# cliangyu/video-diffusion

Measured on AMD Instinct MI355X. Metric: denoise-steps/sec, higher is better.
Workload: dtype f32

## Files before the change

### video-diffusion_amd/csrc/attn_temporal.hip

```cpp
#include "vd_common.h"
#include <cstdlib>
#include <string>

namespace vd {

__device__ __forceinline__ float dot4(f32x4 a, f32x4 b) { return a.x * b.x + a.y * b.y + a.z * b.z + a.w * b.w; }

template <int PB, int TMAX, bool RPE>
__global__ __launch_bounds__(256) void attn_temporal_kernel(AttnTemporalArgs a) {
    extern __shared__ __attribute__((aligned(16))) float smem[];
    const int T = a.T, C = a.C, HW = a.HW, C3 = 3 * a.C;
    const int F = C / a.heads, F4 = F >> 2, FP = F + 4, TS = T + 1;
    float* qs = smem;
    float* ks = qs + PB * T * FP;
    float* sc = ks + PB * T * FP;
    const int b = blockIdx.z, h = blockIdx.y, p0 = blockIdx.x * PB;
    const int np = min(PB, HW - p0);
    const int tid = threadIdx.x;
    const float* qkv_b = a.qkv + (size_t)b * T * HW * C3 + h * F;

    for (int idx = tid; idx < PB * T * F4; idx += 256) {
        const int f4 = idx % F4, r = idx / F4;
        const int t = r % T, p = r / T;
        const float* src = qkv_b + ((size_t)t * HW + p0 + min(p, np - 1)) * C3 + f4 * 4;
        f32x4 q = *reinterpret_cast<const f32x4*>(src) * a.scale;
        f32x4 k = *reinterpret_cast<const f32x4*>(src + C);
        if (p >= np) { q = f32x4{0.f, 0.f, 0.f, 0.f}; k = q; }
        *reinterpret_cast<f32x4*>(qs + (p * T + t) * FP + f4 * 4) = q;
        *reinterpret_cast<f32x4*>(ks + (p * T + t) * FP + f4 * 4) = k;
    }
    __syncthreads();

    for (int pr = tid; pr < T * T; pr += 256) {
        const int t = pr / T, s = pr - t * T;
        float acc[PB];
#pragma unroll
        for (int p = 0; p < PB; ++p) acc[p] = 0.f;
        const float* rk = RPE ? a.Rk + (((size_t)b * T + t) * T + s) * C + h * F : nullptr;
        const float* rq = RPE ? a.Rq + (((size_t)b * T + s) * T + t) * C + h * F : nullptr;
        const float* qrow = qs + t * FP;
        const float* krow = ks + s * FP;
#pragma unroll 3
        for (int f0 = 0; f0 < F; f0 += 8) {
            f32x4 rk0, rk1, rq0, rq1;
            if constexpr (RPE) {
                rk0 = *reinterpret_cast<const f32x4*>(rk + f0); rk1 = *reinterpret_cast<const f32x4*>(rk + f0 + 4);
                rq0 = *reinterpret_cast<const f32x4*>(rq + f0) * a.scale; rq1 = *reinterpret_cast<const f32x4*>(rq + f0 + 4) * a.scale;
            }
#pragma unroll
            for (int p = 0; p < PB; ++p) {
                const f32x4 q0 = *reinterpret_cast<const f32x4*>(qrow + p * T * FP + f0);
                const f32x4 q1 = *reinterpret_cast<const f32x4*>(qrow + p * T * FP + f0 + 4);
                const f32x4 k0 = *reinterpret_cast<const f32x4*>(krow + p * T * FP + f0);
                const f32x4 k1 = *reinterpret_cast<const f32x4*>(krow + p * T * FP + f0 + 4);
                if constexpr (RPE)
                    acc[p] += dot4(q0, k0 + rk0) + dot4(q1, k1 + rk1) + dot4(k0, rq0) + dot4(k1, rq1);
                else
                    acc[p] += dot4(q0, k0) + dot4(q1, k1);
            }
        }
        bool masked = false;
        if (a.mask) {
            const float mt = a.mask[b * T + t], ms = a.mask[b * T + s];
            float allowed = mt * ms;
            if (a.allow_pad) allowed += (1.f - mt) * (1.f - ms);
            else if (t == s) allowed = 1.f;
            masked = allowed == 0.f;
        }
#pragma unroll
        for (int p = 0; p < PB; ++p) sc[(p * T + t) * TS + s] = masked ? -INFINITY : acc[p];
    }
    __syncthreads();

    for (int row = tid; row < np * T; row += 256) {
        float* r = sc + row * TS;
        float mx = -INFINITY;
        for (int s = 0; s < T; ++s) mx = fmaxf(mx, r[s]);
        float sum = 0.f;
        for (int s = 0; s < T; ++s) { const float e = __expf(r[s] - mx); r[s] = e; sum += e; }
        const float inv = 1.0f / sum;
        for (int s = 0; s < T; ++s) r[s] *= inv;
    }
    __syncthreads();

    for (int item = tid; item < T * F4; item += 256) {
        const int t = item / F4, f4 = item - t * F4;
        f32x4 rv[TMAX];
#pragma unroll
        for (int s = 0; s < TMAX; ++s) {
            rv[s] = f32x4{0.f, 0.f, 0.f, 0.f};
            if constexpr (RPE)
                rv[s] = *reinterpret_cast<const f32x4*>(a.Rv + (((size_t)b * T + t) * T + min(s, T - 1)) * C + h * F + f4 * 4);
        }
        for (int p = 0; p < np; ++p) {
            const float* ar = sc + (p * T + t) * TS;
            const float* vbase = qkv_b + 2 * C + (size_t)(p0 + p) * C3 + f4 * 4;
            f32x4 o = {0.f, 0.f, 0.f, 0.f};
#pragma unroll
            for (int s = 0; s < TMAX; ++s) {
                const f32x4 v = *reinterpret_cast<const f32x4*>(vbase + (size_t)min(s, T - 1) * HW * C3);
                const float w = s < T ? ar[min(s, T - 1)] : 0.f;
                o += (v + rv[s]) * w;
            }
            *reinterpret_cast<f32x4*>(a.out + (((size_t)b * T + t) * HW + p0 + p) * C + h * F + f4 * 4) = o;
        }
    }
}

#ifdef VD_ATT_TIMING
__device__ unsigned long long g_att_stamp[16];
#define ATT_STAMP(i)                                                                                   \
    do {                                                                                               \
        if (threadIdx.x == 0 && blockIdx.x == 3 && blockIdx.y == 1 && blockIdx.z == 2) {               \
            __builtin_amdgcn_sched_barrier(0);                                                         \
            g_att_stamp[i] = __builtin_amdgcn_s_memrealtime();                                         \
            __builtin_amdgcn_sched_barrier(0);                                                         \
        }                                                                                              \
    } while (0)
extern "C" int vd_debug_att_stamps(unsigned long long* host_out) {
    return (int)hipMemcpyFromSymbol(host_out, HIP_SYMBOL(g_att_stamp), sizeof(g_att_stamp));
}
#else
#define ATT_STAMP(i)
#endif

__device__ __forceinline__ f32x4 mfma4(float x, float y, f32x4 c) { return __builtin_amdgcn_mfma_f32_16x16x4f32(x, y, c, 0, 0, 0); }

__device__ __forceinline__ void rows_regs_transpose(float& x0, float& x1, float& x2, float& x3) {
    auto u = [](float f) { return __builtin_bit_cast(unsigned, f); };
    auto f = [](unsigned v) { return __builtin_bit_cast(float, v); };
    auto p01 = __builtin_amdgcn_permlane16_swap(u(x0), u(x1), false, false);
    auto p23 = __builtin_amdgcn_permlane16_swap(u(x2), u(x3), false, false);
    auto q02 = __builtin_amdgcn_permlane32_swap(p01[0], p23[0], false, false);
    auto q13 = __builtin_amdgcn_permlane32_swap(p01[1], p23[1], false, false);
    x0 = f(q02[0]); x2 = f(q02[1]); x1 = f(q13[0]); x3 = f(q13[1]);
}

template <int NT, int JM, bool RPE, bool EXACT>
__global__ __launch_bounds__(512, 2) void attn_temporal_mfma_kernel(AttnTemporalArgs a) {
    constexpr int TP = 16 * NT, RS = TP + 1, PS = TP * RS + (NT == 1 ? 1 : 17);
    extern __shared__ __attribute__((aligned(16))) float smem[];
    float* w = smem;
    const int T = EXACT ? 16 * NT : a.T, C = a.C, HW = a.HW, C3 = 3 * a.C;
    const int F = C / a.heads, NJ = EXACT ? JM : F >> 4;
    const int b = blockIdx.z, h = blockIdx.y, p0 = blockIdx.x * 16;
    const int tid = threadIdx.x, wv = tid >> 6, l = tid & 63, i16 = l & 15, g = l >> 4;
    const float* qb = a.qkv + ((size_t)b * T * HW + p0) * C3 + h * F;
    auto row = [&](int t, int px) { return qb + ((size_t)t * HW + px) * C3; };
    auto ld4 = [](const float* p) { return *reinterpret_cast<const f32x4*>(p); };
    const int tcl[2] = {min(i16, T - 1), min(16 + i16, T - 1)};
    const f32x4 zero4 = {0.f, 0.f, 0.f, 0.f};

    ATT_STAMP(0);
    constexpr int JG = NT == 1 ? 2 : 1, NG = JM / JG, NU = 2 * NT;
    constexpr bool AHEAD = NT == 1;
    struct Ops { f32x4 qa1[2][NT][JG], kb1[2][NT][JG], xa2[NU][JG], rb2[NU][NT][JG], xa3[NU][JG], rb3[NU][NT][JG]; };
    f32x4 acc1[2][NT][NT], acc2[NU][NT], acc3[NU][NT];
#pragma unroll
    for (int u = 0; u < 2; ++u)
#pragma unroll
        for (int m = 0; m < NT; ++m)
#pragma unroll
            for (int n = 0; n < NT; ++n) acc1[u][m][n] = zero4;
#pragma unroll
    for (int u = 0; u < NU; ++u)
#pragma unroll
        for (int n = 0; n < NT; ++n) { acc2[u][n] = zero4; acc3[u][n] = zero4; }
    const float* q1[2][NT];
#pragma unroll
    for (int u = 0; u < 2; ++u)
#pragma unroll
        for (int m = 0; m < NT; ++m) q1[u][m] = row(tcl[m], 2 * wv + u) + 4 * g;
    const float* rkq[NT];
#pragma unroll
    for (int n = 0; n < NT; ++n) rkq[n] = (size_t)b * T * T * C + (size_t)tcl[n] * C + h * F + 4 * g + (const float*)nullptr;
    auto request = [&](Ops& o, int grp, bool own, bool rel) {
#pragma unroll
        for (int jj = 0; jj < JG; ++jj) {
            const int j = grp * JG + jj;
            if (EXACT || j < NJ) {
                if (own) {
#pragma unroll
                    for (int u = 0; u < 2; ++u)
#pragma unroll
                        for (int m = 0; m < NT; ++m) { o.qa1[u][m][jj] = ld4(q1[u][m] + 16 * j); o.kb1[u][m][jj] = ld4(q1[u][m] + C + 16 * j); }
                }
                if constexpr (RPE) {
#pragma unroll
                    for (int u = 0; u < (rel ? NU : 0); ++u) {
                        const int t = wv + 8 * u;
                        if (EXACT || t < T) {
                            const float* xr = row(t, i16) + 4 * g + 16 * j;
                            o.xa2[u][jj] = ld4(xr);
                            o.xa3[u][jj] = ld4(xr + C);
#pragma unroll
                            for (int n = 0; n < NT; ++n) {
                                const size_t ro = (size_t)(rkq[n] - (const float*)nullptr) + (size_t)t * T * C + 16 * j;
                                o.rb2[u][n][jj] = ld4(a.Rk + ro);
                                o.rb3[u][n][jj] = ld4(a.Rq + ro);
                            }
                        }
                    }
                }
            }
        }
    };
    auto products = [&](const Ops& o, int grp, bool own, bool rel) {
#pragma unroll
        for (int jj = 0; jj < JG; ++jj) {
            if (EXACT || grp * JG + jj < NJ) {
#pragma unroll
                for (int e = 0; e < 4; ++e) {
#pragma unroll
                    for (int u = 0; u < (own ? 2 : 0); ++u)
#pragma unroll
                        for (int m = 0; m < NT; ++m)
#pragma unroll
                            for (int n = 0; n < NT; ++n) acc1[u][m][n] = mfma4(o.qa1[u][m][jj][e] * a.scale, o.kb1[u][n][jj][e], acc1[u][m][n]);
                    if constexpr (RPE) {
#pragma unroll
                        for (int u = 0; u < (rel ? NU : 0); ++u)
                            if (EXACT || wv + 8 * u < T) {
#pragma unroll
                                for (int n = 0; n < NT; ++n) {
                                    acc2[u][n] = mfma4(o.xa2[u][jj][e] * a.scale, o.rb2[u][n][jj][e], acc2[u][n]);
                                    acc3[u][n] = mfma4(o.xa3[u][jj][e], o.rb3[u][n][jj][e] * a.scale, acc3[u][n]);
                                }
                            }
                    }
                }
            }
        }
    };
    if constexpr (AHEAD) {
        Ops o[2];
        request(o[0], 0, true, true);
#pragma unroll
        for (int grp = 0; grp < NG; ++grp) {
            if (grp + 1 < NG) request(o[(grp + 1) & 1], grp + 1, true, true);
            __builtin_amdgcn_sched_barrier(0);
            products(o[grp & 1], grp, true, true);
            __builtin_amdgcn_sched_barrier(0);
        }
    } else {
#pragma unroll 1
        for (int grp = 0; grp < NG; ++grp) {
            Ops o;
            request(o, grp, true, false);
            products(o, grp, true, false);
            if constexpr (RPE) {
                request(o, grp, false, true);
                products(o, grp, false, true);
            }
        }
    }
    ATT_STAMP(1);
#pragma unroll
    for (int u = 0; u < 2; ++u)
#pragma unroll
        for (int m = 0; m < NT; ++m)
#pragma unroll
            for (int n = 0; n < NT; ++n)
#pragma unroll
                for (int r = 0; r < 4; ++r) w[(2 * wv + u) * PS + (16 * m + 4 * g + r) * RS + 16 * n + i16] = acc1[u][m][n][r];
    __syncthreads();
    if constexpr (RPE) {
#pragma unroll
        for (int u = 0; u < NU; ++u) {
            const int t = wv + 8 * u;
            if (t < T) {
#pragma unroll
                for (int n = 0; n < NT; ++n)
#pragma unroll
                    for (int r = 0; r < 4; ++r) w[(4 * g + r) * PS + t * RS + 16 * n + i16] += acc2[u][n][r];
            }
        }
        __syncthreads();
#pragma unroll
        for (int u = 0; u < NU; ++u) {
            const int sk = wv + 8 * u;
            if (sk < T) {
#pragma unroll
                for (int n = 0; n < NT; ++n)
#pragma unroll
                    for (int r = 0; r < 4; ++r) w[(4 * g + r) * PS + (16 * n + i16) * RS + sk] += acc3[u][n][r];
            }
        }
        __syncthreads();
    }

    ATT_STAMP(2);
    for (int rix = tid; rix < 16 * TP; rix += 512) {
        const int px = rix / TP, t = rix - px * TP;
        float* r = w + px * PS + t * RS;
        if (t >= T) {
            for (int s = 0; s < TP; ++s) r[s] = 0.f;
            continue;
        }
        float mx = -INFINITY;
        const float mt = a.mask ? a.mask[b * T + t] : 1.f;
        for (int s = 0; s < T; ++s) {
            float v = r[s];
            if (a.mask) {
                const float ms = a.mask[b * T + s];
                float allowed = mt * ms;
                if (a.allow_pad) allowed += (1.f - mt) * (1.f - ms);
                else if (t == s) allowed = 1.f;
                if (allowed == 0.f) v = -INFINITY;
            }
            r[s] = v;
            mx = fmaxf(mx, v);
        }
        float sum = 0.f;
        for (int s = 0; s < T; ++s) { const float e = __expf(r[s] - mx); r[s] = e; sum += e; }
        const float inv = 1.0f / sum;
        for (int s = 0; s < T; ++s) r[s] *= inv;
        for (int s = T; s < TP; ++s) r[s] = 0.f;
    }
    __syncthreads();

    ATT_STAMP(3);
    const int KS = (T + 3) >> 2;
    if (EXACT ? wv < JM : wv < NJ) {
        const int f0 = 16 * wv + i16;
        const float* vb = qb + 2 * C + f0;
        const float* rvb = RPE ? a.Rv + ((size_t)b * T) * T * C + h * F + f0 : nullptr;
#pragma unroll 1
        for (int m = 0; m < NT; ++m) {
            if (16 * m >= T) break;
            float rr[NT == 1 ? 4 : 1][16];
            f32x4 acc[16];
#pragma unroll
            for (int px = 0; px < 16; ++px) acc[px] = zero4;
#pragma unroll 1
            for (int kc = 0; kc < NT; ++kc) {
                if (16 * kc >= T) break;
                float vr[4][16];
#pragma unroll
                for (int k4 = 0; k4 < 4; ++k4)
                    if (EXACT || 4 * kc + k4 < KS) {
                        const float* vs = vb + (size_t)min(16 * kc + 4 * k4 + g, T - 1) * HW * C3;
#pragma unroll
                        for (int px = 0; px < 16; ++px) vr[k4][px] = vs[(size_t)px * C3];
                    }
                if constexpr (RPE && NT == 1) {
#pragma unroll
                    for (int k4 = 0; k4 < 4; ++k4)
                        if (EXACT || k4 < KS) {
                            const float* rv = rvb + (size_t)min(4 * k4 + g, T - 1) * C;
#pragma unroll
                            for (int tl = 0; tl < 16; ++tl) rr[k4][tl] = rv[(size_t)min(tl, T - 1) * T * C];
                        }
                }
                __builtin_amdgcn_sched_barrier(0);
#pragma unroll
                for (int k4 = 0; k4 < 4; ++k4)
                    if (EXACT || 4 * kc + k4 < KS) {
                        const float* ar = w + (16 * m + i16) * RS + 16 * kc + 4 * k4 + g;
#pragma unroll
                        for (int px = 0; px < 16; ++px) acc[px] = mfma4(ar[px * PS], vr[k4][px], acc[px]);
                    }
            }
            ATT_STAMP(4);
            f32x4 res[16];
#pragma unroll
            for (int bq = 0; bq < 4; ++bq)
#pragma unroll
                for (int d = 0; d < 4; ++d) {
                    float x0 = acc[bq][d], x1 = acc[4 + bq][d], x2 = acc[8 + bq][d], x3 = acc[12 + bq][d];
                    rows_regs_transpose(x0, x1, x2, x3);
                    res[d][bq] = x0; res[4 + d][bq] = x1; res[8 + d][bq] = x2; res[12 + d][bq] = x3;
                }
            if constexpr (RPE) {
                if constexpr (NT == 1) {
#pragma unroll
                    for (int k4 = 0; k4 < 4; ++k4)
                        if (EXACT || k4 < KS) {
                            const float* ar = w + i16 * PS + 4 * k4 + g;
#pragma unroll
                            for (int tl = 0; tl < 16; ++tl) res[tl] = mfma4(ar[tl * RS], rr[k4][tl], res[tl]);
                        }
                } else {
#pragma unroll 1
                    for (int kc = 0; kc < NT; ++kc) {
                        if (16 * kc >= T) break;
                        float r4[4][16];
#pragma unroll
                        for (int k4 = 0; k4 < 4; ++k4)
                            if (4 * kc + k4 < KS) {
                                const float* rv = rvb + (size_t)min(16 * kc + 4 * k4 + g, T - 1) * C;
#pragma unroll
                                for (int tl = 0; tl < 16; ++tl) r4[k4][tl] = rv[(size_t)min(16 * m + tl, T - 1) * T * C];
                            }
#pragma unroll
                        for (int k4 = 0; k4 < 4; ++k4)
                            if (4 * kc + k4 < KS) {
                                const float* ar = w + i16 * PS + (16 * m) * RS + 16 * kc + 4 * k4 + g;
#pragma unroll
                                for (int tl = 0; tl < 16; ++tl) res[tl] = mfma4(ar[tl * RS], r4[k4][tl], res[tl]);
                            }
                    }
                }
            }
            ATT_STAMP(5);
#pragma unroll
            for (int tl = 0; tl < 16; ++tl) {
                const int t = 16 * m + tl;
                if (t < T) {
                    float* o = a.out + (((size_t)b * T + t) * HW + p0 + 4 * g) * C + h * F + f0;
#pragma unroll
                    for (int r = 0; r < 4; ++r) o[(size_t)r * C] = res[tl][r];
                }
            }
        }
    }
    ATT_STAMP(6);
}

template <int NT, int JM, bool RPE, bool EXACT>
static int launch_tm(const AttnTemporalArgs& a, hipStream_t s) {
    constexpr int TP = 16 * NT, PS = TP * (TP + 1) + (NT == 1 ? 1 : 17);
    constexpr size_t lds = (size_t)16 * PS * sizeof(float);
    if (lds > 48 * 1024) VD_RAISE_LDS((&attn_temporal_mfma_kernel<NT, JM, RPE, EXACT>), lds);
    dim3 grid(a.HW / 16, a.heads, a.B);
    hipLaunchKernelGGL((attn_temporal_mfma_kernel<NT, JM, RPE, EXACT>), grid, dim3(512), lds, s, a);
    VD_HIP(hipGetLastError());
    return 0;
}

template <int PB, int TMAX, bool RPE>
static int launch_tt(const AttnTemporalArgs& a, size_t lds, hipStream_t s) {
    VD_RAISE_LDS((&attn_temporal_kernel<PB, TMAX, RPE>), lds);
    dim3 grid((a.HW + PB - 1) / PB, a.heads, a.B);
    hipLaunchKernelGGL((attn_temporal_kernel<PB, TMAX, RPE>), grid, dim3(256), lds, s, a);
    VD_HIP(hipGetLastError());
    return 0;
}

AttnTemporalVariant attn_temporal_variant(int T, int HW, int C, int heads, bool rpe) {
    using V = AttnTemporalVariant;
    V v{V::kRefused, 0, 0, false, rpe, 0, nullptr};
    auto pick = [&](V::Family fam, int p0, int p1, bool exact, size_t lds) { v.family = fam; v.p0 = p0; v.p1 = p1; v.exact = exact; v.lds = lds; return v; };
    if (!(T >= 1 && T <= kMaxWindowFrames)) { v.why = "temporal window of 1..128 frames"; return v; }
    if (!(heads > 0 && C > 0 && C % heads == 0 && (C / heads) % 8 == 0)) { v.why = "head dim multiple of 8"; return v; }
    const int F = C / heads;
    const bool pipe = HW % 16 == 0 && F % 16 == 0 && F <= 128;
    if (T > 32)
        return pipe ? pick(V::kLongMfma, F / 16, 0, false, 0) : pick(V::kLongGeneric, 0, 0, false, 0);
    if (pipe) {
        if (T == 16 && F == 96) return pick(V::kMfma, 1, 6, true, 0);
        if (T == 16 && F == 128) return pick(V::kMfma, 1, 8, true, 0);
        return pick(V::kMfma, T <= 16 ? 1 : 2, F <= 64 ? 4 : 8, false, 0);
    }
    auto lds_for = [&](int pb) { return ((size_t)2 * pb * T * (F + 4) + (size_t)pb * T * (T + 1)) * sizeof(float); };
    if (!(lds_for(2) <= 150 * 1024)) { v.why = "head dim too large for the temporal attention tile"; return v; }
    const int pb = lds_for(4) > 96 * 1024 ? 2 : 4;
    return pick(V::kValu, pb, T <= 16 ? 16 : 32, false, lds_for(pb));
}

std::string attn_temporal_variant_name(const AttnTemporalVariant& v) {
    using V = AttnTemporalVariant;
    const char* r = v.rpe ? "true" : "false";
    const std::string p0 = std::to_string(v.p0), p1 = std::to_string(v.p1);
    switch (v.family) {
        case V::kMfma: return "attn_temporal_mfma_kernel<" + p0 + "," + p1 + "," + r + "," + (v.exact ? "true" : "false") + ">";
        case V::kValu: return "attn_temporal_kernel<" + p0 + "," + p1 + "," + r + ">";
        case V::kLongMfma: return "attn_temporal_long_mfma_kernel<" + p0 + "," + r + ">";
        case V::kLongGeneric: return std::string("attn_temporal_long_kernel<") + r + ">";
        default: return std::string("refused: ") + (v.why ? v.why : "");
    }
}

template <bool RPE>
static int launch_variant(const AttnTemporalVariant& v, const AttnTemporalArgs& a, hipStream_t s) {
    if (v.family == AttnTemporalVariant::kMfma) {
        if (v.exact) return v.p1 == 6 ? launch_tm<1, 6, RPE, true>(a, s) : launch_tm<1, 8, RPE, true>(a, s);
        if (v.p0 == 1) return v.p1 == 4 ? launch_tm<1, 4, RPE, false>(a, s) : launch_tm<1, 8, RPE, false>(a, s);
        return v.p1 == 4 ? launch_tm<2, 4, RPE, false>(a, s) : launch_tm<2, 8, RPE, false>(a, s);
    }
    if (v.p1 == 16) return v.p0 == 2 ? launch_tt<2, 16, RPE>(a, v.lds, s) : launch_tt<4, 16, RPE>(a, v.lds, s);
    return v.p0 == 2 ? launch_tt<2, 32, RPE>(a, v.lds, s) : launch_tt<4, 32, RPE>(a, v.lds, s);
}

int launch_attn_temporal(const AttnTemporalArgs& a, hipStream_t s) {
    const bool rpe = a.Rk != nullptr;
    const AttnTemporalVariant v = attn_temporal_variant(a.T, a.HW, a.C, a.heads, rpe);
    VD_REQUIRE(v.family != AttnTemporalVariant::kRefused, v.why);
    VD_REQUIRE((a.Rk == nullptr) == (a.Rq == nullptr) && (a.Rk == nullptr) == (a.Rv == nullptr), "all or no RPE terms");
    if (v.family == AttnTemporalVariant::kLongMfma || v.family == AttnTemporalVariant::kLongGeneric) return launch_attn_temporal_long(a, s);
    return rpe ? launch_variant<true>(v, a, s) : launch_variant<false>(v, a, s);
}

}
```

Before: 51.25.

## Stage Q/K tiles through LDS in temporal MFMA attention instead of per-wave global loads

```diff
diff --git a/video-diffusion_amd/csrc/attn_temporal.hip b/video-diffusion_amd/csrc/attn_temporal.hip
--- a/video-diffusion_amd/csrc/attn_temporal.hip
+++ b/video-diffusion_amd/csrc/attn_temporal.hip
@@ -152,9 +152,14 @@
     const f32x4 zero4 = {0.f, 0.f, 0.f, 0.f};
 
     ATT_STAMP(0);
-    constexpr int JG = NT == 1 ? 2 : 1, NG = JM / JG, NU = 2 * NT;
+    constexpr int JG = NT == 1 && (RPE || EXACT) ? 2 : 1, NG = JM / JG, NU = 2 * NT;
     constexpr bool AHEAD = NT == 1;
-    struct Ops { f32x4 qa1[2][NT][JG], kb1[2][NT][JG], xa2[NU][JG], rb2[NU][NT][JG], xa3[NU][JG], rb3[NU][NT][JG]; };
+    constexpr int SF = 16 * JG, LPR = SF / 4, RSQ = SF + 8, FS = 16 * RSQ + 8;
+    constexpr int NLD = 16 * TP * LPR / 512, TSTEP = 512 / (16 * LPR);
+    static_assert(NLD * TSTEP == TP, "512 threads cover the stage in NLD passes");
+    float* sq = smem;
+    float* sk = smem + TP * FS;
+    struct Rb { f32x4 rb2[NU][NT][JG], rb3[NU][NT][JG]; };
     f32x4 acc1[2][NT][NT], acc2[NU][NT], acc3[NU][NT];
 #pragma unroll
     for (int u = 0; u < 2; ++u)
@@ -166,33 +171,44 @@
     for (int u = 0; u < NU; ++u)
 #pragma unroll
         for (int n = 0; n < NT; ++n) { acc2[u][n] = zero4; acc3[u][n] = zero4; }
-    const float* q1[2][NT];
-#pragma unroll
-    for (int u = 0; u < 2; ++u)
-#pragma unroll
-        for (int m = 0; m < NT; ++m) q1[u][m] = row(tcl[m], 2 * wv + u) + 4 * g;
+    const int scc = 4 * (tid % LPR), spx = (tid / LPR) & 15, st0 = tid / (16 * LPR);
+    auto srow = [&](int i) { return row(min(st0 + TSTEP * i, T - 1), spx); };
+    const float* gs[AHEAD ? NLD : 1];
+#pragma unroll
+    for (int i = 0; i < (AHEAD ? NLD : 0); ++i) gs[i] = srow(i);
+    const int sdst = st0 * FS + spx * RSQ + scc;
+    f32x4 sr[2][NLD];
+    auto fetch = [&](int grp) {
+        const int co = EXACT ? SF * grp + scc : min(SF * grp + scc, F - 4);
+#pragma unroll
+        for (int i = 0; i < NLD; ++i) {
+            const float* r = AHEAD ? gs[AHEAD ? i : 0] : srow(i);
+            sr[0][i] = ld4(r + co);
+            sr[1][i] = ld4(r + C + co);
+        }
+    };
+    auto commit = [&]() {
+#pragma unroll
+        for (int i = 0; i < NLD; ++i) {
+            *reinterpret_cast<f32x4*>(sq + sdst + i * TSTEP * FS) = sr[0][i];
+            *reinterpret_cast<f32x4*>(sk + sdst + i * TSTEP * FS) = sr[1][i];
+        }
+    };
+    const int fo1 = i16 * FS + 2 * wv * RSQ + 4 * g;
+    const int fo2 = wv * FS + i16 * RSQ + 4 * g;
     const float* rkq[NT];
 #pragma unroll
     for (int n = 0; n < NT; ++n) rkq[n] = (size_t)b * T * T * C + (size_t)tcl[n] * C + h * F + 4 * g + (const float*)nullptr;
-    auto request = [&](Ops& o, int grp, bool own, bool rel) {
-#pragma unroll
-        for (int jj = 0; jj < JG; ++jj) {
-            const int j = grp * JG + jj;
-            if (EXACT || j < NJ) {
-                if (own) {
-#pragma unroll
-                    for (int u = 0; u < 2; ++u)
-#pragma unroll
-                        for (int m = 0; m < NT; ++m) { o.qa1[u][m][jj] = ld4(q1[u][m] + 16 * j); o.kb1[u][m][jj] = ld4(q1[u][m] + C + 16 * j); }
-                }
-                if constexpr (RPE) {
-#pragma unroll
-                    for (int u = 0; u < (rel ? NU : 0); ++u) {
+    auto request = [&](Rb& o, int grp) {
+        if constexpr (RPE) {
+#pragma unroll
+            for (int jj = 0; jj < JG; ++jj) {
+                const int j = grp * JG + jj;
+                if (EXACT || j < NJ) {
+#pragma unroll
+                    for (int u = 0; u < NU; ++u) {
                         const int t = wv + 8 * u;
                         if (EXACT || t < T) {
-                            const float* xr = row(t, i16) + 4 * g + 16 * j;
-                            o.xa2[u][jj] = ld4(xr);
-                            o.xa3[u][jj] = ld4(xr + C);
 #pragma unroll
                             for (int n = 0; n < NT; ++n) {
                                 const size_t ro = (size_t)(rkq[n] - (const float*)nullptr) + (size_t)t * T * C + 16 * j;
@@ -205,10 +221,25 @@
             }
         }
     };
-    auto products = [&](const Ops& o, int grp, bool own, bool rel) {
+    auto products = [&](const Rb& o, int grp, bool own, bool rel) {
 #pragma unroll
         for (int jj = 0; jj < JG; ++jj) {
             if (EXACT || grp * JG + jj < NJ) {
+                f32x4 qa1[2][NT], kb1[2][NT], xa2[NU], xa3[NU];
+#pragma unroll
+                for (int u = 0; u < (own ? 2 : 0); ++u)
+#pragma unroll
+                    for (int m = 0; m < NT; ++m) {
+                        qa1[u][m] = ld4(sq + fo1 + 16 * m * FS + u * RSQ + 16 * jj);
+                        kb1[u][m] = ld4(sk + fo1 + 16 * m * FS + u * RSQ + 16 * jj);
+                    }
+                if constexpr (RPE) {
+#pragma unroll
+                    for (int u = 0; u < (rel ? NU : 0); ++u) {
+                        xa2[u] = ld4(sq + fo2 + 8 * u * FS + 16 * jj);
+                        xa3[u] = ld4(sk + fo2 + 8 * u * FS + 16 * jj);
+                    }
+                }
 #pragma unroll
                 for (int e = 0; e < 4; ++e) {
 #pragma unroll
@@ -216,15 +247,15 @@
 #pragma unroll
                         for (int m = 0; m < NT; ++m)
 #pragma unroll
-                            for (int n = 0; n < NT; ++n) acc1[u][m][n] = mfma4(o.qa1[u][m][jj][e] * a.scale, o.kb1[u][n][jj][e], acc1[u][m][n]);
+                            for (int n = 0; n < NT; ++n) acc1[u][m][n] = mfma4(qa1[u][m][e] * a.scale, kb1[u][n][e], acc1[u][m][n]);
                     if constexpr (RPE) {
 #pragma unroll
                         for (int u = 0; u < (rel ? NU : 0); ++u)
                             if (EXACT || wv + 8 * u < T) {
 #pragma unroll
                                 for (int n = 0; n < NT; ++n) {
-                                    acc2[u][n] = mfma4(o.xa2[u][jj][e] * a.scale, o.rb2[u][n][jj][e], acc2[u][n]);
-                                    acc3[u][n] = mfma4(o.xa3[u][jj][e], o.rb3[u][n][jj][e] * a.scale, acc3[u][n]);
+                                    acc2[u][n] = mfma4(xa2[u][e] * a.scale, o.rb2[u][n][jj][e], acc2[u][n]);
+                                    acc3[u][n] = mfma4(xa3[u][e], o.rb3[u][n][jj][e] * a.scale, acc3[u][n]);
                                 }
                             }
                     }
@@ -233,25 +264,36 @@
         }
     };
     if constexpr (AHEAD) {
-        Ops o[2];
-        request(o[0], 0, true, true);
+        Rb o[2];
+        fetch(0);
+        request(o[0], 0);
+        commit();
+        __syncthreads();
 #pragma unroll
         for (int grp = 0; grp < NG; ++grp) {
-            if (grp + 1 < NG) request(o[(grp + 1) & 1], grp + 1, true, true);
-            __builtin_amdgcn_sched_barrier(0);
-            products(o[grp & 1], grp, true, true);
-            __builtin_amdgcn_sched_barrier(0);
+            if (EXACT || grp * JG < NJ) {
+                const bool more = grp + 1 < NG && (EXACT || (grp + 1) * JG < NJ);
+                if (more) { fetch(grp + 1); request(o[(grp + 1) & 1], grp + 1); }
+                __builtin_amdgcn_sched_barrier(0);
+                products(o[grp & 1], grp, true, true);
+                __builtin_amdgcn_sched_barrier(0);
+                __syncthreads();
+                if (more) { commit(); __syncthreads(); }
+            }
         }
     } else {
 #pragma unroll 1
         for (int grp = 0; grp < NG; ++grp) {
-            Ops o;
-            request(o, grp, true, false);
+            if (grp * JG >= NJ) break;
+            Rb o;
+            fetch(grp);
+            commit();
+            request(o, grp);
+            __syncthreads();
             products(o, grp, true, false);
-            if constexpr (RPE) {
-                request(o, grp, false, true);
-                products(o, grp, false, true);
-            }
+            __builtin_amdgcn_sched_barrier(0);
+            products(o, grp, false, true);
+            __syncthreads();
         }
     }
     ATT_STAMP(1);
@@ -420,8 +462,10 @@
 template <int NT, int JM, bool RPE, bool EXACT>
 static int launch_tm(const AttnTemporalArgs& a, hipStream_t s) {
     constexpr int TP = 16 * NT, PS = TP * (TP + 1) + (NT == 1 ? 1 : 17);
-    constexpr size_t lds = (size_t)16 * PS * sizeof(float);
-    if (lds > 48 * 1024) VD_RAISE_LDS((&attn_temporal_mfma_kernel<NT, JM, RPE, EXACT>), lds);
+    constexpr int SF = NT == 1 && (RPE || EXACT) ? 32 : 16, FS = 16 * (SF + 8) + 8;
+    constexpr size_t lds_w = (size_t)16 * PS * sizeof(float), lds_s = (size_t)2 * TP * FS * sizeof(float), lds = lds_w > lds_s ? lds_w : lds_s;
+    static_assert(lds <= 160 * 1024, "LDS of one CU");
+    VD_RAISE_LDS((&attn_temporal_mfma_kernel<NT, JM, RPE, EXACT>), lds);
     dim3 grid(a.HW / 16, a.heads, a.B);
     hipLaunchKernelGGL((attn_temporal_mfma_kernel<NT, JM, RPE, EXACT>), grid, dim3(512), lds, s, a);
     VD_HIP(hipGetLastError());
```

Result: no change. 51.39, median of 6 (+0.3%).
